# kouyt5/lightning-asr

Measured on AMD Instinct MI355X. Metric: audio-seconds/sec training (asr13x1, bs=32, 10 s clips), higher is better.
Workload: dtype bf16; 1 GPU; asr13x1 QuartzNet-CTC train step, bs=32/GPU, 10 s synthetic 16 kHz clips, labels.txt vocab (C=28), HIP mel+conv+CTC+NovoGrad, random-init weights; global_batch=32, n_class=28, parallelism=dp1, feature_prefetch=True, hip_graph=True, staged_backward=False

## Files before the change

include/lasr.h:

```cpp
#ifndef LASR_H
#define LASR_H

#include <stddef.h>
#include <stdint.h>

#ifdef __cplusplus
extern "C" {
#endif

#define LASR_VERSION 108

enum { LASR_F32 = 0, LASR_BF16 = 1 };
enum { LASR_ACT_NONE = 0, LASR_ACT_RELU = 1, LASR_ACT_SWISH = 2 };
enum { LASR_VARIANT_PLAIN = 0, LASR_VARIANT_CONTEXT = 1, LASR_VARIANT_CONTEXT_SE = 2 };
enum {
  LASR_E_ARG = -1,
  LASR_E_SHAPE = -2,
  LASR_E_WORKSPACE = -3,
  LASR_E_FORMAT = -4,
  LASR_E_UNSUPPORTED = -5,
  LASR_E_IO = -6
};

int lasr_version(void);
const char* lasr_last_error(void);

int64_t lasr_mel_num_frames(int64_t n_samples);
size_t lasr_mel_workspace_bytes(int64_t B, int64_t T);
int lasr_mel_fwd(const float* wave, const int32_t* sample_lens, const float* dither, const int32_t* aug,
                 int64_t B, int64_t L, int normalize, float* out_bft, void* out_btf, int dtype,
                 int32_t* frames_out, float* pct_out, void* workspace, size_t workspace_bytes, void* stream);

#define LASR_LEN_LEAD (1 << 30)
enum { LASR_WAVE_F32 = 0, LASR_WAVE_PCM16 = 1 };
typedef struct {
  const void* wave; int32_t wave_dtype; const float* dither; uint64_t dither_seed; uint64_t* dither_step; int64_t pitch;
} lasr_wave_src;
int lasr_mel_fwd_src(const lasr_wave_src* src, const int32_t* sample_lens, const int32_t* aug, int64_t B, int64_t L,
                     int normalize, float* out_bft, void* out_btf, int dtype, int32_t* frames_out, float* pct_out,
                     void* workspace, size_t workspace_bytes, void* stream);
int lasr_dither_noise(uint64_t seed, const uint64_t* step, int64_t B, int64_t L, float* out, void* stream);

int lasr_spec_augment(const float* in, float* out, const int32_t* aug, int64_t B, int64_t F, int64_t T, void* stream);

int lasr_bct_to_btc(const float* in, void* out, int dtype, int64_t B, int64_t C, int64_t T, void* stream);
int lasr_btc_to_bct(const void* in, int dtype, float* out, int64_t B, int64_t C, int64_t T, void* stream);

int lasr_mask_lengths(const float* pct, int64_t B, int64_t T, int32_t* lens, void* stream);


int lasr_dwconv_fwd(const void* x, const float* w, const void* addend, void* y, int dtype, int64_t B,
                    int64_t Tin, int64_t C, int k, int stride, int flip, void* stream);
size_t lasr_dwconv_wgrad_workspace_bytes(int64_t B, int64_t Tout, int64_t C, int k);
int lasr_dwconv_wgrad(const void* x, const void* dy, float* dw, int dtype, int64_t B, int64_t Tin,
                      int64_t C, int k, int stride, void* workspace, size_t workspace_bytes, void* stream);

size_t lasr_gemm_workspace_bytes(int64_t M, int64_t N, int split_k, int want_stats);
int lasr_gemm(const void* A, const void* B, void* C, int dtype_ab, int dtype_c, int64_t M, int64_t N,
              int64_t K, int transA, int transB, const float* bias, const void* addend,
              const int32_t* row_lens, int64_t rows_per_seq, float* stats, int split_k, void* workspace,
              size_t workspace_bytes, void* stream);

typedef struct {
  const void* A; const void* B; void* C;
  int64_t M, N, K;
  const float* bias; const int32_t* row_lens; int64_t rows_per_seq; float* stats;
} lasr_gemm_problem;
size_t lasr_gemm_batch_workspace_bytes(const lasr_gemm_problem* probs, int n_probs, int split_k);
int lasr_gemm_batch(const lasr_gemm_problem* probs, int n_probs, int dtype_ab, int dtype_c, int transA, int transB,
                    int split_k, void* workspace, size_t workspace_bytes, void* stream);

int lasr_gemm_ld(const void* A, int64_t lda, const void* B, int64_t ldb, void* C, int64_t ldc, int dtype_ab, int dtype_c,
                 int64_t M, int64_t N, int64_t K, int transA, int transB, const float* bias, int split_k, void* workspace,
                 size_t workspace_bytes, void* stream);

typedef struct {
  const float* w; const float* w_res; const float* coef; const float* coef2; void* w_out; float* bias_out; int64_t co, ci;
} lasr_fold_desc;
int lasr_fold_bn_weights_many(const lasr_fold_desc* descs, int n_descs, void* stream);
int lasr_gemm_dual(const void* A1, int64_t K1, const void* A2, int64_t K2, const void* W, const float* bias, void* C,
                   int64_t M, int64_t N, const int32_t* row_lens, int64_t rows_per_seq, int act, void* stream);

typedef struct { const float* partials; float* out; int64_t n; int32_t n_partials; } lasr_reduce_desc;
int lasr_reduce_many(const lasr_reduce_desc* descs, int n_descs, void* stream);
int lasr_gemm_batch_split_partials(const lasr_gemm_problem* probs, int n_probs, int dtype_ab, int transA, int transB,
                                   int split_k, void* workspace, size_t workspace_bytes, const float** partials,
                                   int* splits, void* stream);
int lasr_gemm_multi_split_partials(const lasr_gemm_problem* probs, int n_probs, int split_k, float* const* slabs,
                                   int* splits, void* stream);
int lasr_dwconv_wgrad_partials(const void* x, const void* dy, int dtype, int64_t B, int64_t Tin, int64_t C, int k,
                               int stride, void* workspace, size_t workspace_bytes, int* n_partials, void* stream);
int lasr_dwconv_bwd_fused(const void* x, const void* dy, const float* w, const void* addend, void* dx, int dtype,
                          int64_t B, int64_t T, int64_t C, int k, void* workspace, size_t workspace_bytes,
                          int* n_partials, void* stream);

int lasr_gemm_batch_partials(const lasr_gemm_problem* probs, int n_probs, int dtype_ab, int dtype_c, int transA,
                             int transB, void* workspace, size_t workspace_bytes, const float** stat_partials,
                             int* stat_tiles, void* stream);

int lasr_bn_finalize(const float* stats, const float* gamma, const float* beta, float* running_mean,
                     float* running_var, float* coef, float* saved, int64_t C, int64_t n_rows, float eps,
                     float momentum, int training, void* stream);
typedef struct {
  const float* gamma; const float* beta; const float* running_mean; const float* running_var; float* coef; int64_t C;
} lasr_bn_eval_desc;
int lasr_bn_eval_coef_many(const lasr_bn_eval_desc* descs, int n_descs, float eps, void* stream);

typedef struct {
  const float* partials; int n_partials;
  const float* gamma; const float* beta; float* running_mean; float* running_var;
  float* coef; float* saved; float* stats;
} lasr_bn_branch;
int lasr_bn_finalize_partials(const lasr_bn_branch* branches, int n_branches, int64_t C, int64_t n_rows, float eps,
                              float momentum, void* stream);
// ... 265 lines not shown
```

lightning_asr_amd/_lib.py:

```python
from __future__ import annotations

import ctypes as C
import os

_HERE = os.path.dirname(os.path.abspath(__file__))
LIB_PATH = os.environ.get("LASR_LIB_PATH", os.path.join(_HERE, "liblasr.so"))

F32, BF16 = 0, 1
ACT_NONE, ACT_RELU, ACT_SWISH = 0, 1, 2
LEN_LEAD = 1 << 30
VARIANT = {"plain": 0, "context": 1, "context_se": 2}

_p, _i64, _i32, _f32, _sz = C.c_void_p, C.c_int64, C.c_int, C.c_float, C.c_size_t


class Dropout(C.Structure):
    _fields_ = [("step", C.c_void_p), ("seed", C.c_uint64), ("unit", C.c_uint32), ("p", C.c_float)]


class WaveSrc(C.Structure):
    _fields_ = [("wave", C.c_void_p), ("wave_dtype", C.c_int32), ("dither", C.c_void_p), ("dither_seed", C.c_uint64),
                ("dither_step", C.c_void_p), ("pitch", C.c_int64)]


WAVE_F32, WAVE_PCM16 = 0, 1


class ModelConfig(C.Structure):
    _fields_ = [("variant", C.c_int32), ("n_class", C.c_int32), ("in_c", C.c_int32),
                ("mask", C.c_int32), ("act", C.c_int32), ("dtype", C.c_int32)]


SIGNATURES = {
    "lasr_version": (_i32, []),
    "lasr_roctx_range_push": (_i32, [C.c_char_p]),
    "lasr_roctx_range_pop": (_i32, []),
    "lasr_roctx_enabled": (_i32, []),
    "lasr_last_error": (C.c_char_p, []),
    "lasr_mel_num_frames": (_i64, [_i64]),
    "lasr_mel_workspace_bytes": (_sz, [_i64, _i64]),
    "lasr_mel_fwd": (_i32, [_p, _p, _p, _p, _i64, _i64, _i32, _p, _p, _i32, _p, _p, _p, _sz, _p]),
    "lasr_mel_fwd_src": (_i32, [_p, _p, _p, _i64, _i64, _i32, _p, _p, _i32, _p, _p, _p, _sz, _p]),
    "lasr_dither_noise": (_i32, [C.c_uint64, _p, _i64, _i64, _p, _p]),
    "lasr_spec_augment": (_i32, [_p, _p, _p, _i64, _i64, _i64, _p]),
    "lasr_bct_to_btc": (_i32, [_p, _p, _i32, _i64, _i64, _i64, _p]),
    "lasr_btc_to_bct": (_i32, [_p, _i32, _p, _i64, _i64, _i64, _p]),
    "lasr_mask_lengths": (_i32, [_p, _i64, _i64, _p, _p]),
    "lasr_dwconv_fwd": (_i32, [_p, _p, _p, _p, _i32, _i64, _i64, _i64, _i32, _i32, _i32, _p]),
    "lasr_dwconv_wgrad_workspace_bytes": (_sz, [_i64, _i64, _i64, _i32]),
    "lasr_dwconv_wgrad": (_i32, [_p, _p, _p, _i32, _i64, _i64, _i64, _i32, _i32, _p, _sz, _p]),
    "lasr_gemm_workspace_bytes": (_sz, [_i64, _i64, _i32, _i32]),
    "lasr_gemm": (_i32, [_p, _p, _p, _i32, _i32, _i64, _i64, _i64, _i32, _i32, _p, _p, _p, _i64, _p, _i32, _p, _sz, _p]),
    "lasr_gemm_batch_workspace_bytes": (_sz, [_p, _i32, _i32]),
    "lasr_gemm_batch": (_i32, [_p, _i32, _i32, _i32, _i32, _i32, _i32, _p, _sz, _p]),
    "lasr_bn_finalize": (_i32, [_p, _p, _p, _p, _p, _p, _p, _i64, _i64, _f32, _f32, _i32, _p]),
    "lasr_bn_eval_coef_many": (_i32, [_p, _i32, _f32, _p]),
    "lasr_bn_act_fwd": (_i32, [_p, _p, _p, _p, _p, _p, _i32, _i64, _i64, _i64, _i32, _p]),
    "lasr_bn_bwd_workspace_bytes": (_sz, [_i64, _i64, _i64]),
    "lasr_bn_act_bwd_stats": (_i32, [_p] * 11 + [_i32, _i64, _i64, _i64, _i32, _p, _sz, _p]),
    "lasr_bn_act_bwd_apply": (_i32, [_p] * 20 + [_i32, _i64, _i64, _i64, _i32, _p, _sz, _p]),
    "lasr_bn_bwd_apply_workspace_bytes": (_sz, [_i64]),
    "lasr_reduce_many": (_i32, [_p, _i32, _p]),
    "lasr_gemm_batch_split_partials": (_i32, [_p, _i32, _i32, _i32, _i32, _i32, _p, _sz, _p, _p, _p]),
    "lasr_gemm_multi_split_partials": (_i32, [_p, _i32, _i32, _p, _p, _p]),
    "lasr_dwconv_wgrad_partials": (_i32, [_p, _p, _i32, _i64, _i64, _i64, _i32, _i32, _p, _sz, _p, _p]),
    "lasr_dwconv_bwd_fused": (_i32, [_p, _p, _p, _p, _p, _i32, _i64, _i64, _i64, _i32, _p, _sz, _p, _p]),
    "lasr_gemm_batch_partials": (_i32, [_p, _i32, _i32, _i32, _i32, _i32, _p, _sz, _p, _p, _p]),
    "lasr_bn_finalize_partials": (_i32, [_p, _i32, _i64, _i64, C.c_float, C.c_float, _p]),
    "lasr_bn_act_fwd_partials": (_i32, [_p, _i32, C.c_float, C.c_float, _p, _p, _p, _i32, _i64, _i64, _i64, _i32, _p]),
    "lasr_seqsum": (_i32, [_p, _i32, _i64, _i64, _i64, _p, _p]),
    "lasr_se_fwd": (_i32, [_p, _p, _p, _p, _i64, _i64, _i64, _p, _p, _p, _p]),
    "lasr_se_bwd_workspace_bytes": (_sz, [_i64, _i64]),
    "lasr_se_bwd": (_i32, [_p] * 10 + [_i32, _i64, _i64, _i64, _i32, _p, _p, _p, _p, _sz, _p]),
    "lasr_bilstm_saved_bytes": (_sz, [_i64, _i64]),
    "lasr_bilstm_fwd": (_i32, [_p] * 9 + [_i64, _i64, _p, _i32, _i64, _i64, _p, _p]),
    "lasr_bilstm_bwd_workspace_bytes": (_sz, [_i64]),
    "lasr_bilstm_bwd": (_i32, [_p, _i32, _i64, _i64, _p, _p, _p, _i64, _i64, _p, _p, _p, _p, _p, _p, _sz, _p]),
    "lasr_copy_cols": (_i32, [_p, _i32, _i64, _i64, _p, _i32, _i64, _i64, _i64, _i64, _i32, _p]),
    "lasr_log_softmax": (_i32, [_p, _p, _p, _i64, _i64, _p]),
    "lasr_log_softmax_bwd": (_i32, [_p, _p, _p, _i64, _i64, _p]),
    "lasr_ctc_workspace_bytes": (_sz, [_i64, _i64, _i64]),
    "lasr_ctc_loss": (_i32, [_p, _p, _p, _p, _i64, _i64, _i64, _i64, _i32, _p, _p, _p, _p, _sz, _p]),
    "lasr_ctc_loss_mel": (_i32, [_p, _p, _p, _p, _i64, _i64, _i64, _i64, _i32, _p, _p, _p, _p, _sz,
                                 _p, _p, _p, _p, _i64, _i64, _i32, _p, _p, _i32, _p, _p, _p, _sz, _p]),
    "lasr_ctc_align_workspace_bytes": (_sz, [_i64, _i64, _i64]),
    "lasr_ctc_align": (_i32, [_p, _p, _p, _p, _i64, _i64, _i64, _i64, _i32, _p, _p, _p, _p, _p, _p, _sz, _p]),
    "lasr_greedy_decode": (_i32, [_p, _p, _i64, _i64, _i32, _p, _p, _p]),
    "lasr_ctc_beam_workspace_bytes": (_sz, [_i64, _i64, _i64, _i32, _i32]),
    "lasr_ctc_beam_decode": (_i32, [_p, _p, _i64, _i64, _i64, _i32, _i32, _i32, _f32, _i32, _p, _p, _p, _p, _sz, _p]),
    "lasr_arpa_load": (_i32, [C.c_char_p, _p, _i32, C.POINTER(_p)]),
    "lasr_arpa_info": (_i32, [_p, C.POINTER(C.c_int), C.POINTER(C.c_int), C.POINTER(_i64), C.POINTER(_sz)]),
    "lasr_arpa_write_image": (_i32, [_p, _p, _sz]),
    "lasr_arpa_free": (None, [_p]),
    "lasr_ctc_beam_lm_workspace_bytes": (_sz, [_i64, _i64, _i64, _i32, _i32]),
    "lasr_ctc_beam_decode_lm": (_i32, [_p, _p, _i64, _i64, _i64, _i32, _i32, _i32, _f32, _i32, _p, _f32, _f32, _p, _p, _p, _p, _p, _sz,
                                       _p]),
    "lasr_arpa_load_words": (_i32, [C.c_char_p, _p, _i32, _i32, C.POINTER(_p)]),
    "lasr_arpa_lexicon_info": (_i32, [_p, C.POINTER(_i64), C.POINTER(_i64), C.POINTER(_i64)]),
    "lasr_ctc_beam_decode_wlm": (_i32, [_p, _p, _i64, _i64, _i64, _i32, _i32, _i32, _f32, _i32, _p, _f32, _f32, _p, _p, _p, _p, _p, _sz,
                                        _p]),
    "lasr_novograd_workspace_bytes": (_sz, [_i64, _i64]),
    "lasr_novograd_step": (_i32, [_p, _p, _p, _p, _p, _i64, _i64, _p, _f32, _f32, _f32, _f32, _f32, _p, _sz, _p]),
    "lasr_novograd_step_keep": (_i32, [_p, _p, _p, _p, _p, _i64, _i64, _p, _f32, _f32, _f32, _f32, _f32, _p, _sz, _p]),
    "lasr_cast_f32_to_bf16": (_i32, [_p, _p, _i64, _p]),
    "lasr_cast_pad_f32_to_bf16": (_i32, [_p, _p, _i64, _i64, _i64, _p]),
# ... 105 lines not shown
```

lightning_asr_amd/csrc/gemm.h:

```cpp
#pragma once
#include "common.h"

namespace lasr {

struct GemmArgs {
  const void* A; const void* B; void* C;
  int64_t M, N, K, lda, ldb, ldc;
  const float* bias; const void* addend;
  const int32_t* row_lens; int64_t rows_per_seq;
  float* stat_partials;
  float* split_ws;
  int64_t k_per_split;
  int vecA, vecB;
};

int launch_gemm_bf16(const GemmArgs& g, int gz, int dtype_c, int transA, int transB, hipStream_t st, int* stat_tiles);
int launch_gemm_bf16_batch(const GemmArgs* g, const int* gz, int n, int dtype_c, int transA, int transB, hipStream_t st,
                           int* stat_tiles);

int launch_gemm_bf16_dual(const GemmArgs& g, const void* A2, int64_t lda2, int64_t K1, const float* bias, int act, hipStream_t st);
namespace lstm { struct BwdArgs; }
int launch_gemm_bf16_multi(const GemmArgs* g, const int* gz, int n, bool big_tile, hipStream_t st, const lstm::BwdArgs* lstm_job = nullptr,
                           int lstm_wgs = 0, const lasr_reduce_desc* riders = nullptr, int n_riders = 0, int* riders_taken = nullptr);
int gemm_multi_split_partials_riders(const lasr_gemm_problem* probs, int n_probs, int split_k, float* const* slabs, int* splits,
                                     const lasr_reduce_desc* riders, int n_riders, int* riders_taken, void* stream);
int gemm_split_partials_one(const void* A, const void* B, int dtype_ab, int64_t M, int64_t N, int64_t K, int transA, int transB, int split_k,
                            void* workspace, size_t workspace_bytes, int* splits, void* stream);
int gemm_multi_split_partials_with_bilstm_bwd(const lasr_gemm_problem* probs, int n_probs, int* n_taken, int split_k, float* const* slabs, int* splits,
                                              const lstm::BwdArgs& rec, int dtype, int64_t B, void* stream);
int launch_gemm_bf16_rowstat(const GemmArgs& g, float* row_stat, int32_t* row_arg, int* n_col_tiles, hipStream_t st);

}
```

lightning_asr_amd/csrc/gemm.hip:

```cpp
#include "common.h"
#include "gemm.h"
#include "lstm_body.h"
#include <cmath>
#include <climits>
#include <stdlib.h>

namespace lasr {

typedef float f32x16 __attribute__((ext_vector_type(16)));

static constexpr int BM = 128, BN = 128, BK = 16;
static constexpr int LDS_LD = BM + 4;

template <typename T, bool TRANS>
__device__ __forceinline__ void load_tile(const T* __restrict__ X, int64_t ld, int64_t R, int64_t K, int64_t r0, int64_t k0,
                                          int64_t kend, bool vec_ok, float (&reg)[2][4]) {
  const int tid = threadIdx.x;
#pragma unroll
  for (int p = 0; p < 2; ++p) {
    reg[p][0] = reg[p][1] = reg[p][2] = reg[p][3] = 0.f;
    if (!TRANS) {
      const int64_t r = r0 + (tid >> 2) + 64 * p;
      const int64_t k = k0 + ((tid & 3) << 2);
      if (r < R) {
// ... 169 lines not shown
                                                                int64_t ldc, const float* __restrict__ bias,
                                                                const TC* __restrict__ addend, TC* __restrict__ C) {
  const int64_t i = blockIdx.x * (int64_t)blockDim.x + threadIdx.x;
  if (i >= M * N) return;
  const int64_t m = i / N, n = i - m * N;
  float s = 0.f;
  for (int p = 0; p < split; ++p) s += ws[(int64_t)p * M * N + i];
  if (bias) s += bias[n];
  if (addend) s += Elem<TC>::ld(addend + m * ldc + n);
  Elem<TC>::st(C + m * ldc + n, s);
}

struct SplitReduce2 { const float* ws[2]; float* C[2]; const float* bias[2]; int split[2]; int64_t M[2], N[2]; };
__global__ __launch_bounds__(256) void gemm_split_reduce2_kernel(SplitReduce2 a) {
  const int q = blockIdx.y;
  const int64_t i = blockIdx.x * (int64_t)blockDim.x + threadIdx.x;
  const int64_t mn = a.M[q] * a.N[q];
  if (i >= mn) return;
  const float* ws = a.ws[q];
  float s = 0.f;
  for (int p = 0; p < a.split[q]; ++p) s += ws[(int64_t)p * mn + i];
  if (a.bias[q]) s += a.bias[q][i % a.N[q]];
  a.C[q][i] = s;
}

template <typename TAB, typename TC>
static int launch_f32(const GemmArgs& g, int transA, int transB, dim3 grid, hipStream_t st) {
#define LASR_GEMM_CASE(TA_, TB_)                                                                              \
  hipLaunchKernelGGL((gemm_f32_kernel<TAB, TC, TA_, TB_>), grid, dim3(256), 0, st, g)
  if (!transA && !transB) LASR_GEMM_CASE(false, false);
  else if (!transA && transB) LASR_GEMM_CASE(false, true);
  else if (transA && !transB) LASR_GEMM_CASE(true, false);
  else LASR_GEMM_CASE(true, true);
#undef LASR_GEMM_CASE
  LASR_LAUNCH_CHECK("gemm_f32_kernel");
  return 0;
}

}

using namespace lasr;

extern "C" size_t lasr_gemm_workspace_bytes(int64_t M, int64_t N, int split_k, int want_stats) {
  size_t b = 0;
  if (split_k > 1) b += align_up((size_t)split_k * M * N * sizeof(float), 256);
  if (want_stats) b += align_up((size_t)cdiv(M, BM) * 2 * N * sizeof(float), 256);
  return b;
}

struct StatOut { const float* partials; int tiles; };
static int gemm_impl(const void* A, const void* B, void* C, int dtype_ab, int dtype_c, int64_t M, int64_t N, int64_t K,
                     int transA, int transB, const float* bias, const void* addend, const int32_t* row_lens,
                     int64_t rows_per_seq, float* stats, int split_k, void* workspace, size_t workspace_bytes,
                     void* stream, StatOut* stat_out, int64_t lda = 0, int64_t ldb = 0, int64_t ldc = 0, int* split_left_out = nullptr) {
  LASR_CHECK_ARG(A && B && C, "lasr_gemm: null pointer");
  LASR_CHECK_ARG((dtype_ab == LASR_F32 || dtype_ab == LASR_BF16) && (dtype_c == LASR_F32 || dtype_c == LASR_BF16), "lasr_gemm: bad dtype");
  LASR_CHECK_SHAPE(M > 0 && N > 0 && K > 0 && split_k >= 1 && split_k <= 1024, "lasr_gemm: M=%lld N=%lld K=%lld split=%d",
                   (long long)M, (long long)N, (long long)K, split_k);
  LASR_CHECK_ARG(!(row_lens && rows_per_seq <= 0), "lasr_gemm: rows_per_seq");
  LASR_CHECK_ARG(!(split_k > 1 && (row_lens || stats)), "lasr_gemm: split_k excludes masking/statistics");
  const size_t need = lasr_gemm_workspace_bytes(M, N, split_k, stats != nullptr);
  if (need > 0 && (!workspace || workspace_bytes < need)) return fail(LASR_E_WORKSPACE, "lasr_gemm: workspace %zu < %zu", workspace_bytes, need);
  GemmArgs g;
  g.A = A; g.B = B; g.C = C; g.M = M; g.N = N; g.K = K;
  g.lda = lda > 0 ? lda : (transA ? M : K); g.ldb = ldb > 0 ? ldb : (transB ? N : K); g.ldc = ldc > 0 ? ldc : N;
  LASR_CHECK_SHAPE(g.lda >= (transA ? M : K) && g.ldb >= (transB ? N : K) && g.ldc >= N, "lasr_gemm: leading dimension smaller than the row");
  g.bias = bias; g.addend = addend; g.row_lens = row_lens; g.rows_per_seq = rows_per_seq;
  g.stat_partials = nullptr; g.split_ws = nullptr;
  const size_t esz = dtype_size(dtype_ab);
  const bool addend_ok = addend == nullptr || (dtype_c == LASR_BF16 && N % 4 == 0 && g.ldc % 4 == 0 && reinterpret_cast<uintptr_t>(addend) % 8 == 0);
  const bool use_bf16 = dtype_ab == LASR_BF16 && addend_ok && !getenv("LASR_FORCE_F32_MFMA");
  const int vw = use_bf16 ? 8 : 4;
  g.vecA = (g.lda % vw == 0) && (reinterpret_cast<uintptr_t>(A) % (vw * esz) == 0);
  g.vecB = (g.ldb % vw == 0) && (reinterpret_cast<uintptr_t>(B) % (vw * esz) == 0);
  char* wsp = reinterpret_cast<char*>(workspace);
  if (split_k > 1) {
    g.split_ws = reinterpret_cast<float*>(wsp);
    wsp += align_up((size_t)split_k * M * N * sizeof(float), 256);
    const int64_t per = cdiv(cdiv(K, split_k), 64) * 64;
    g.k_per_split = per;
    split_k = (int)cdiv(K, per);
  } else {
    g.k_per_split = K;
  }
  int grid_m = (int)cdiv(M, BM);
  if (stats) g.stat_partials = reinterpret_cast<float*>(wsp);
  dim3 grid((unsigned)cdiv(N, BN), (unsigned)grid_m, (unsigned)split_k);
  hipStream_t st = as_stream(stream);
  const double gbytes = (double)(M * K + N * K) * esz + (double)M * N * dtype_size(dtype_c);
  const int tok = prof_begin(LASR_PROF_GEMM, st, 2.0 * (double)M * (double)N * (double)K, gbytes);
  int rc;
  if (use_bf16) rc = launch_gemm_bf16(g, split_k, dtype_c, transA, transB, st, &grid_m);
  else if (dtype_ab == LASR_F32) rc = dtype_c == LASR_F32 ? launch_f32<float, float>(g, transA, transB, grid, st) : launch_f32<float, bf16_t>(g, transA, transB, grid, st);
  else rc = dtype_c == LASR_F32 ? launch_f32<bf16_t, float>(g, transA, transB, grid, st) : launch_f32<bf16_t, bf16_t>(g, transA, transB, grid, st);
  prof_end(tok, st);
  if (rc) return rc;
  if (g.split_ws && split_left_out) {
    *split_left_out = split_k;
  } else if (g.split_ws) {
    const int64_t mn = M * N;
    if (dtype_c == LASR_F32)
      hipLaunchKernelGGL(gemm_split_reduce_kernel<float>, dim3((unsigned)cdiv(mn, 256)), dim3(256), 0, st, g.split_ws, split_k, M, N, g.ldc, bias, (const float*)addend, (float*)C);
    else
      hipLaunchKernelGGL(gemm_split_reduce_kernel<bf16_t>, dim3((unsigned)cdiv(mn, 256)), dim3(256), 0, st, g.split_ws, split_k, M, N, g.ldc, bias, (const bf16_t*)addend, (bf16_t*)C);
    LASR_LAUNCH_CHECK("gemm_split_reduce_kernel");
  }
  if (stats && stat_out) {
    stat_out->partials = g.stat_partials; stat_out->tiles = grid_m;
  } else if (stats) {
    LASR_TRY(launch_reduce_partials(g.stat_partials, grid_m, 2 * N, stats, 2 * N, nullptr, st));
  }
  return 0;
}

int lasr::gemm_split_partials_one(const void* A, const void* B, int dtype_ab, int64_t M, int64_t N, int64_t K, int transA, int transB,
                                  int split_k, void* workspace, size_t workspace_bytes, int* splits, void* stream) {
  LASR_CHECK_ARG(splits && split_k > 1 && workspace, "gemm_split_partials_one: bad argument");
  return gemm_impl(A, B, workspace , dtype_ab, LASR_F32, M, N, K, transA, transB, nullptr, nullptr, nullptr,
                   0, nullptr, split_k, workspace, workspace_bytes, stream, nullptr, 0, 0, 0, splits);
}

extern "C" int lasr_gemm_ld(const void* A, int64_t lda, const void* B, int64_t ldb, void* C, int64_t ldc, int dtype_ab, int dtype_c,
                            int64_t M, int64_t N, int64_t K, int transA, int transB, const float* bias, int split_k, void* workspace,
                            size_t workspace_bytes, void* stream) {
  return gemm_impl(A, B, C, dtype_ab, dtype_c, M, N, K, transA, transB, bias, nullptr, nullptr, 0, nullptr, split_k, workspace,
                   workspace_bytes, stream, nullptr, lda, ldb, ldc);
}

extern "C" int lasr_gemm(const void* A, const void* B, void* C, int dtype_ab, int dtype_c, int64_t M, int64_t N, int64_t K,
                         int transA, int transB, const float* bias, const void* addend, const int32_t* row_lens,
                         int64_t rows_per_seq, float* stats, int split_k, void* workspace, size_t workspace_bytes,
                         void* stream) {
  return gemm_impl(A, B, C, dtype_ab, dtype_c, M, N, K, transA, transB, bias, addend, row_lens, rows_per_seq, stats, split_k,
                   workspace, workspace_bytes, stream, nullptr);
}

extern "C" int lasr_gemm_rowstat(const void* A, const void* B, const float* bias, void* C, int64_t ldc, int64_t M, int64_t N, int64_t K,
                                 float* row_stat, int32_t* row_arg, int* n_col_tiles, void* stream) {
  LASR_CHECK_ARG(A && B && C && row_stat && row_arg, "lasr_gemm_rowstat: null pointer");
  LASR_CHECK_SHAPE(M > 0 && N > 0 && K > 0 && K % 8 == 0 && ldc >= N && ldc % 8 == 0, "lasr_gemm_rowstat: M=%lld N=%lld K=%lld ldc=%lld",
                   (long long)M, (long long)N, (long long)K, (long long)ldc);
  GemmArgs g;
  g.A = A; g.B = B; g.C = C; g.M = M; g.N = N; g.K = K; g.lda = K; g.ldb = K; g.ldc = ldc;
  g.bias = bias; g.addend = nullptr; g.row_lens = nullptr; g.rows_per_seq = 0; g.stat_partials = nullptr; g.split_ws = nullptr;
  g.k_per_split = K;
  g.vecA = reinterpret_cast<uintptr_t>(A) % 16 == 0; g.vecB = reinterpret_cast<uintptr_t>(B) % 16 == 0;
  hipStream_t st = as_stream(stream);
  const int tok = prof_begin(LASR_PROF_GEMM, st, 2.0 * (double)M * N * K, (double)(M * K + N * K) * 2 + (double)M * N * 2);
  const int rc = launch_gemm_bf16_rowstat(g, row_stat, row_arg, n_col_tiles, st);
  prof_end(tok, st);
  return rc;
}
extern "C" size_t lasr_gemm_rowstat_bytes(int64_t M, int64_t N) { return (size_t)M * cdiv(N, 256) * (2 * sizeof(float) + sizeof(int32_t)); }

extern "C" size_t lasr_gemm_batch_workspace_bytes(const lasr_gemm_problem* probs, int n_probs, int split_k) {
  size_t b = 0;
  for (int i = 0; i < n_probs; ++i) b += lasr_gemm_workspace_bytes(probs[i].M, probs[i].N, split_k, probs[i].stats != nullptr);
  return b;
}

struct SplitOut { const float* partials; int splits; };
static int gemm_batch_impl(const lasr_gemm_problem* probs, int n_probs, int dtype_ab, int dtype_c, int transA, int transB,
                           int split_k, void* workspace, size_t workspace_bytes, void* stream, StatOut* stat_out,
                           SplitOut* split_out = nullptr) {
  LASR_CHECK_ARG(probs && n_probs >= 1 && n_probs <= 2, "lasr_gemm_batch: 1 or 2 problems");
  const size_t need = lasr_gemm_batch_workspace_bytes(probs, n_probs, split_k);
  if (need > 0 && (!workspace || workspace_bytes < need)) return fail(LASR_E_WORKSPACE, "lasr_gemm_batch: workspace %zu < %zu", workspace_bytes, need);
  char* wsp = reinterpret_cast<char*>(workspace);
  if (split_out && (dtype_ab != LASR_BF16 || n_probs == 1))
    return fail(LASR_E_ARG, "lasr_gemm_batch_split_partials: two bf16 problems per call");
  if (dtype_ab != LASR_BF16 || n_probs == 1 || getenv("LASR_NO_GEMM_BATCH")) {
    for (int i = 0; i < n_probs; ++i) {
      const lasr_gemm_problem& q = probs[i];
      const size_t nb = lasr_gemm_workspace_bytes(q.M, q.N, split_k, q.stats != nullptr);
      LASR_TRY(gemm_impl(q.A, q.B, q.C, dtype_ab, dtype_c, q.M, q.N, q.K, transA, transB, q.bias, nullptr, q.row_lens, q.rows_per_seq,
                         q.stats, split_k, wsp, nb, stream, stat_out ? stat_out + i : nullptr));
      wsp += nb;
    }
    return 0;
  }
  LASR_CHECK_ARG(dtype_c == LASR_F32 || dtype_c == LASR_BF16, "lasr_gemm_batch: bad dtype");
  GemmArgs g[2];
  int splits[2], stat_tiles[2];
  for (int i = 0; i < 2; ++i) {
    const lasr_gemm_problem& q = probs[i];
    LASR_CHECK_ARG(q.A && q.B && q.C, "lasr_gemm_batch: null pointer");
    LASR_CHECK_SHAPE(q.M > 0 && q.N > 0 && q.K > 0 && split_k >= 1 && split_k <= 1024, "lasr_gemm_batch: shape");
// ... 237 lines not shown
```

lightning_asr_amd/csrc/gemm_bf16.hip:

```cpp
#include "gemm.h"
#include "reduce_body.h"
#include "lstm_body.h"
#include <algorithm>
#include <stdlib.h>

namespace lasr {

__device__ __forceinline__ void load_bias_quads(const float* __restrict__ bias, int nbase, int N, float (&bv)[4][4]) {
#pragma unroll
  for (int ni = 0; ni < 4; ++ni)
#pragma unroll
    for (int e = 0; e < 4; ++e) {
      const int n = nbase + ni * 16 + e;
      bv[ni][e] = __uint_as_float(__float_as_uint(bias[min(n, N - 1)]) & (n < N ? 0xffffffffu : 0u));
    }
}


typedef float f32x4 __attribute__((ext_vector_type(4)));
typedef __bf16 bf16x8 __attribute__((ext_vector_type(8)));
typedef short s16x4 __attribute__((ext_vector_type(4)));
typedef short s16x8 __attribute__((ext_vector_type(8)));

static constexpr int TM = 128, TN = 128, TK = 64;
static constexpr int LD_KC = 144;
static constexpr int LD_RC = 320;
static constexpr int OPER_BYTES = 20480;
static constexpr int EPI_LD = 144;

union Frag { uint4 u; s16x8 s; bf16x8 b; };

struct Bf16Args {
  const bf16_t* A; const bf16_t* B; void* C;
  const float* bias; const int32_t* row_lens; float* stat_partials; float* split_ws;
  const bf16_t* addend;
  int M, N, K, lda, ldb, ldc, rows_per_seq, k_per_split;
  int gm, gn, gz;
  int vecA, vecB, vecC;
  const bf16_t* A2; int lda2, K1, act;
  float* row_stat; int32_t* row_arg;
};
struct Bf16Batch { Bf16Args p[2]; int tiles0, total; };

__device__ __forceinline__ int kc_slot(int row, int ch) { return ch ^ (((row >> 2) ^ (row >> 3)) & 1); }

__device__ __forceinline__ uint4 mask_chunk(const uint4& v, int nvalid) {
  const int n = max(0, min(nvalid, 8));
  if (n == 8) return v;
  auto dm = [n](int i) -> uint32_t { return n >= 2 * i + 2 ? 0xffffffffu : (n == 2 * i + 1 ? 0x0000ffffu : 0u); };
  return make_uint4(v.x & dm(0), v.y & dm(1), v.z & dm(2), v.w & dm(3));
}

template <bool TRANS, int ROWS, int NT, int NCH = 4, bool NTL = false>
// ... 733 lines not shown

template <bool NTL>
__global__ __launch_bounds__(512, 1) void gemm_bf16_big_multi_kernel(Bf16Multi gm) {
  if ((int)blockIdx.x >= gm.total) {
    const int r = blockIdx.x - gm.total;
    for (int s = 0; s < gm.n_rd; ++s) {
      const lasr_reduce_desc q = gm.rd[s];
      for (int64_t i = (int64_t)r * big::NT + threadIdx.x; i < q.n; i += (int64_t)gm.n_rwg * big::NT) reduce_many_elem(q, i);
    }
    return;
  }
  const int lid_all = xcd_remap(blockIdx.x, gm.total);
  int i = 0;
  while (i + 1 < gm.n && gm.start[i + 1] <= lid_all) ++i;
  gemm_bf16_big_tile<true, true, false, true, false, NTL>(gm.p[i], lid_all - gm.start[i]);
}

struct LstmJob { lstm::BwdArgs a; int n_wg; int n_utt; };
template <bool NTL, int KP, bool PAIR>
__global__ __launch_bounds__(512, 1) void gemm_bf16_big_multi_lstm_kernel(Bf16Multi gm, LstmJob job) {
  if ((int)blockIdx.x < job.n_wg) {
    __shared__ lstm::BwdSmem sm[2];
    const int slot = threadIdx.x / 192;
    if (slot >= (PAIR ? 2 : 1)) return;
    const int b = PAIR ? blockIdx.x : blockIdx.x >> 1, dir = PAIR ? slot : (blockIdx.x & 1);
    lstm::bilstm_bwd_body<bf16_t, true, KP>(job.a, b, dir, (int)threadIdx.x - slot * 192, 192, sm[slot], [] { lds_barrier(); });
    return;
  }
  const int lid_all = xcd_remap((int)blockIdx.x - job.n_wg, gm.total);
  int i = 0;
  while (i + 1 < gm.n && gm.start[i + 1] <= lid_all) ++i;
  gemm_bf16_big_tile<true, true, false, true, false, NTL>(gm.p[i], lid_all - gm.start[i]);
}

static int fill_args(Bf16Args& a, const GemmArgs& g, int tm, int tn, int gz) {
  const int64_t lim = (int64_t)1 << 31;
  const int64_t gn = cdiv(g.N, tn), gm = cdiv(g.M, tm);
  if (g.M * g.lda >= lim || g.K * g.lda >= lim || g.N * g.ldb >= lim || g.K * g.ldb >= lim || g.M * g.ldc >= lim ||
      gn * gm * gz >= lim / 2)
    return fail(LASR_E_SHAPE, "lasr_gemm(bf16): matrix exceeds the kernel's 32-bit element offsets");
  a.A = reinterpret_cast<const bf16_t*>(g.A); a.B = reinterpret_cast<const bf16_t*>(g.B); a.C = g.C;
  a.bias = g.bias; a.row_lens = g.row_lens; a.stat_partials = g.stat_partials; a.split_ws = g.split_ws;
  a.M = (int)g.M; a.N = (int)g.N; a.K = (int)g.K; a.lda = (int)g.lda; a.ldb = (int)g.ldb; a.ldc = (int)g.ldc;
  a.rows_per_seq = (int)(g.rows_per_seq > 0 ? g.rows_per_seq : 1); a.k_per_split = (int)g.k_per_split;
  a.gn = (int)gn; a.gm = (int)gm; a.gz = gz;
  a.vecA = g.vecA; a.vecB = g.vecB;
  a.vecC = (g.ldc % 8 == 0) && (reinterpret_cast<uintptr_t>(g.C) % 16 == 0);
  a.A2 = nullptr; a.lda2 = 0; a.K1 = 0; a.act = 0;
  a.row_stat = nullptr; a.row_arg = nullptr;
  a.addend = reinterpret_cast<const bf16_t*>(g.addend);
  return 0;
}

int launch_gemm_bf16_batch(const GemmArgs* g, const int* gz, int n, int dtype_c, int transA, int transB, hipStream_t st,
                           int* stat_tiles) {
  const bool f32_out = dtype_c == LASR_F32 || g[0].split_ws != nullptr;
  static const int big_min = getenv("LASR_GEMM_BIG_MIN_TILES") ? atoi(getenv("LASR_GEMM_BIG_MIN_TILES")) : 120;
  int64_t nmax = 0;
  for (int i = 0; i < n; ++i) nmax = std::max<int64_t>(nmax, g[i].N);
  static const bool force_narrow = getenv("LASR_GEMM_FORCE_NARROW") && atoi(getenv("LASR_GEMM_FORCE_NARROW")) != 0;
  const bool narrow = nmax <= 256 || force_narrow;
  const int btn = narrow ? 128 : 256;
  int64_t big_tiles = 0;
  for (int i = 0; i < n; ++i) big_tiles += cdiv(g[i].M, big::BTM) * cdiv(g[i].N, btn) * gz[i];
  bool vec = true;
  for (int i = 0; i < n; ++i) vec = vec && g[i].vecA && g[i].vecB;
  bool has_add = false;
  for (int i = 0; i < n; ++i) has_add = has_add || g[i].addend != nullptr;
  const bool use_big = !f32_out && vec && big_tiles >= big_min && !has_add;
  const int tm = use_big ? big::BTM : TM, tn = use_big ? btn : TN;
  Bf16Batch b;
  LASR_TRY(fill_args(b.p[0], g[0], tm, tn, gz[0]));
  b.p[1] = b.p[0];
  if (n > 1) LASR_TRY(fill_args(b.p[1], g[1], tm, tn, gz[1]));
  b.tiles0 = b.p[0].gn * b.p[0].gm * b.p[0].gz;
  b.total = b.tiles0 + (n > 1 ? b.p[1].gn * b.p[1].gm * b.p[1].gz : 0);
  if (stat_tiles)
    for (int i = 0; i < n; ++i) stat_tiles[i] = b.p[i].gm;
  const dim3 grid1((unsigned)b.total);
  if (use_big) {
#define LASR_BIG_CASE(TA_, TB_)                                                                              \
  do {                                                                                                     \
    if (narrow) hipLaunchKernelGGL((gemm_bf16_big_kernel<TA_, TB_, true>), grid1, dim3(big::NT), 0, st, b);  \
    else hipLaunchKernelGGL((gemm_bf16_big_kernel<TA_, TB_, false>), grid1, dim3(big::NT), 0, st, b);        \
  } while (0)
    if (!transA && !transB) LASR_BIG_CASE(false, false);
    else if (!transA && transB) LASR_BIG_CASE(false, true);
    else if (transA && !transB) LASR_BIG_CASE(true, false);
    else LASR_BIG_CASE(true, true);
#undef LASR_BIG_CASE
    LASR_LAUNCH_CHECK("gemm_bf16_big_kernel");
    return 0;
  }
#define LASR_BF16_CASE(TC_, TA_, TB_)                                                                    \
  do {                                                                                                  \
    if (vec) hipLaunchKernelGGL((gemm_bf16_kernel<TC_, TA_, TB_, true>), grid1, dim3(256), 0, st, b);    \
    else hipLaunchKernelGGL((gemm_bf16_kernel<TC_, TA_, TB_, false>), grid1, dim3(256), 0, st, b);       \
  } while (0)
#define LASR_BF16_TC(TC_)                                         \
  do {                                                            \
    if (!transA && !transB) LASR_BF16_CASE(TC_, false, false);    \
    else if (!transA && transB) LASR_BF16_CASE(TC_, false, true); \
    else if (transA && !transB) LASR_BF16_CASE(TC_, true, false); \
    else LASR_BF16_CASE(TC_, true, true);                         \
  } while (0)
  if (f32_out) LASR_BF16_TC(float); else LASR_BF16_TC(bf16_t);
#undef LASR_BF16_TC
#undef LASR_BF16_CASE
  LASR_LAUNCH_CHECK("gemm_bf16_kernel");
  return 0;
}

int launch_gemm_bf16_dual(const GemmArgs& g, const void* A2, int64_t lda2, int64_t K1, const float* bias, int act, hipStream_t st) {
  if (K1 <= 0 || K1 >= g.K || K1 % TK || (g.K - K1) % TK || lda2 % 8 || g.lda % 8 || g.ldb % 8 || g.ldc % 8 ||
      reinterpret_cast<uintptr_t>(g.A) % 16 || reinterpret_cast<uintptr_t>(A2) % 16 || reinterpret_cast<uintptr_t>(g.B) % 16 ||
      reinterpret_cast<uintptr_t>(g.C) % 16 || !bias)
    return fail(LASR_E_SHAPE, "lasr_gemm_dual: K parts must be multiples of %d, pitches of 8, pointers 16-byte aligned, bias given", TK);
  Bf16Batch b;
  LASR_TRY(fill_args(b.p[0], g, big::BTM, 128, 1));
  b.p[0].A2 = reinterpret_cast<const bf16_t*>(A2); b.p[0].lda2 = (int)lda2; b.p[0].K1 = (int)K1; b.p[0].act = act;
  b.p[0].bias = bias;
  b.p[1] = b.p[0];
  b.tiles0 = b.p[0].gn * b.p[0].gm;
  b.total = b.tiles0;
  hipLaunchKernelGGL(gemm_bf16_dual_kernel, dim3((unsigned)b.total), dim3(big::NT), 0, st, b);
  LASR_LAUNCH_CHECK("gemm_bf16_dual_kernel");
  return 0;
}

// ... 19 lines not shown
  Bf16Multi m;
  m.n_rd = 0; m.n_rwg = 0;
  bool vec = true;
  int total = 0;
  for (int i = 0; i < n; ++i) {
    if (!g[i].split_ws) return fail(LASR_E_ARG, "lasr_gemm_multi_split_partials: every problem needs a slab buffer");
    LASR_TRY(fill_args(m.p[i], g[i], big_tile ? big::BTM : TM, big_tile ? 256 : TN, gz[i]));
    vec = vec && g[i].vecA && g[i].vecB;
    m.start[i] = total;
    total += m.p[i].gn * m.p[i].gm * m.p[i].gz;
  }
  for (int i = n; i < kMaxMulti; ++i) m.p[i] = m.p[0];
  for (int i = n; i <= kMaxMulti; ++i) m.start[i] = total;
  m.n = n; m.total = total;
  if (big_tile) {
    if (!vec) return fail(LASR_E_ARG, "lasr_gemm_multi_split_partials: the 256-row tile needs 16-byte aligned operand rows");
    if (lstm_job) {
      static const bool pair = getenv("LASR_LSTM_PAIR") && atoi(getenv("LASR_LSTM_PAIR")) == 1;
      LstmJob job; job.a = *lstm_job; job.n_wg = lstm_wgs; job.n_utt = pair ? lstm_wgs : lstm_wgs / 2;
      if (job.n_wg % 8) return fail(LASR_E_SHAPE, "gemm + BiLSTM grid: the batch must be a multiple of 8 utterances");
      if (pair) hipLaunchKernelGGL((gemm_bf16_big_multi_lstm_kernel<false, 16, true>), dim3((unsigned)(total + job.n_wg)), dim3(big::NT), 0, st, m, job);
      else hipLaunchKernelGGL((gemm_bf16_big_multi_lstm_kernel<false, 16, false>), dim3((unsigned)(total + job.n_wg)), dim3(big::NT), 0, st, m, job);
      LASR_LAUNCH_CHECK("gemm_bf16_big_multi_lstm_kernel");
      return 0;
    }
    static const bool riders_off = getenv("LASR_WGRAD_RIDERS") && atoi(getenv("LASR_WGRAD_RIDERS")) == 0;
    const int idle = 256 - total;
    if (!riders_off && riders && riders_taken && n_riders > 0 && idle >= 8) {
      int ksteps = 0;
      for (int i = 0; i < n; ++i) ksteps = std::max(ksteps, (int)cdiv(m.p[i].k_per_split, 64));
      double budget = (double)idle * 20e9 * ((double)ksteps * 1.7e-6 + 20e-6) * 0.8;
      while (m.n_rd < n_riders && m.n_rd < kMaxRiders) {
        const lasr_reduce_desc& q = riders[m.n_rd];
        const double bytes = (double)q.n * (q.n_partials + 1) * sizeof(float);
        if (bytes > budget) break;
        budget -= bytes;
        m.rd[m.n_rd++] = q;
      }
      if (m.n_rd > 0) { m.n_rwg = idle; *riders_taken = m.n_rd; }
    }
    for (int i = m.n_rd; i < kMaxRiders; ++i) m.rd[i] = lasr_reduce_desc{nullptr, nullptr, 0, 0};
    if (nt_loads_mask() & 8) hipLaunchKernelGGL(gemm_bf16_big_multi_kernel<true>, dim3((unsigned)(total + m.n_rwg)), dim3(big::NT), 0, st, m);
    else hipLaunchKernelGGL(gemm_bf16_big_multi_kernel<false>, dim3((unsigned)(total + m.n_rwg)), dim3(big::NT), 0, st, m);
    LASR_LAUNCH_CHECK("gemm_bf16_big_multi_kernel");
    return 0;
  }
  if (lstm_job) return fail(LASR_E_SHAPE, "gemm + BiLSTM grid needs the 256-row tile form");
  if (vec) hipLaunchKernelGGL(gemm_bf16_multi_kernel<true>, dim3((unsigned)total), dim3(256), 0, st, m);
  else hipLaunchKernelGGL(gemm_bf16_multi_kernel<false>, dim3((unsigned)total), dim3(256), 0, st, m);
  LASR_LAUNCH_CHECK("gemm_bf16_multi_kernel");
  return 0;
}

int launch_gemm_bf16(const GemmArgs& g, int gz, int dtype_c, int transA, int transB, hipStream_t st, int* stat_tiles) {
  return launch_gemm_bf16_batch(&g, &gz, 1, dtype_c, transA, transB, st, stat_tiles);
}

}

#ifdef LASR_GEMM_STAMPS
extern "C" int lasr_debug_set_gemm_stamps(void* buf) {
  unsigned long long* p = reinterpret_cast<unsigned long long*>(buf);
  return (int)hipMemcpyToSymbol(HIP_SYMBOL(lasr::g_stamps), &p, sizeof(p));
}
#endif
```

Before: 160,300 audio-seconds/sec.

## Choose bf16 GEMM tile family with a wave-count cost model

Replaces the fixed heuristic for picking the GEMM tile shape (128x128, 256x128, 256x256), which used a tile-count threshold and an N cutoff, with a cost model. The model estimates waves over the device's CU count times per-tile fixed and per-K-step costs. It switches away from the old choice only when the predicted saving clears a margin, and it keeps the old choice for GEMMs that emit BN statistics. A new lasr_gemm_tile entry point allows forcing a tile family. The risk is that hand-fit cost constants may misjudge some shapes and pick a slower tile.

```diff
diff --git a/include/lasr.h b/include/lasr.h
--- a/include/lasr.h
+++ b/include/lasr.h
@@ -60,6 +60,9 @@
               int64_t K, int transA, int transB, const float* bias, const void* addend,
               const int32_t* row_lens, int64_t rows_per_seq, float* stats, int split_k, void* workspace,
               size_t workspace_bytes, void* stream);
+int lasr_gemm_tile(const void* A, const void* B, void* C, int dtype_ab, int dtype_c, int64_t M, int64_t N,
+                   int64_t K, int transA, int transB, const float* bias, const int32_t* row_lens,
+                   int64_t rows_per_seq, float* stats, int tile, void* workspace, size_t workspace_bytes, void* stream);
 
 typedef struct {
   const void* A; const void* B; void* C;
diff --git a/lightning_asr_amd/_lib.py b/lightning_asr_amd/_lib.py
--- a/lightning_asr_amd/_lib.py
+++ b/lightning_asr_amd/_lib.py
@@ -51,6 +51,7 @@
     "lasr_dwconv_wgrad": (_i32, [_p, _p, _p, _i32, _i64, _i64, _i64, _i32, _i32, _p, _sz, _p]),
     "lasr_gemm_workspace_bytes": (_sz, [_i64, _i64, _i32, _i32]),
     "lasr_gemm": (_i32, [_p, _p, _p, _i32, _i32, _i64, _i64, _i64, _i32, _i32, _p, _p, _p, _i64, _p, _i32, _p, _sz, _p]),
+    "lasr_gemm_tile": (_i32, [_p, _p, _p, _i32, _i32, _i64, _i64, _i64, _i32, _i32, _p, _p, _i64, _p, _i32, _p, _sz, _p]),
     "lasr_gemm_batch_workspace_bytes": (_sz, [_p, _i32, _i32]),
     "lasr_gemm_batch": (_i32, [_p, _i32, _i32, _i32, _i32, _i32, _i32, _p, _sz, _p]),
     "lasr_bn_finalize": (_i32, [_p, _p, _p, _p, _p, _p, _p, _i64, _i64, _f32, _f32, _i32, _p]),
diff --git a/lightning_asr_amd/csrc/gemm.h b/lightning_asr_amd/csrc/gemm.h
--- a/lightning_asr_amd/csrc/gemm.h
+++ b/lightning_asr_amd/csrc/gemm.h
@@ -14,9 +14,9 @@
   int vecA, vecB;
 };
 
-int launch_gemm_bf16(const GemmArgs& g, int gz, int dtype_c, int transA, int transB, hipStream_t st, int* stat_tiles);
+int launch_gemm_bf16(const GemmArgs& g, int gz, int dtype_c, int transA, int transB, hipStream_t st, int* stat_tiles, int force_tile = 0);
 int launch_gemm_bf16_batch(const GemmArgs* g, const int* gz, int n, int dtype_c, int transA, int transB, hipStream_t st,
-                           int* stat_tiles);
+                           int* stat_tiles, int force_tile = 0);
 
 int launch_gemm_bf16_dual(const GemmArgs& g, const void* A2, int64_t lda2, int64_t K1, const float* bias, int act, hipStream_t st);
 namespace lstm { struct BwdArgs; }
diff --git a/lightning_asr_amd/csrc/gemm.hip b/lightning_asr_amd/csrc/gemm.hip
--- a/lightning_asr_amd/csrc/gemm.hip
+++ b/lightning_asr_amd/csrc/gemm.hip
@@ -245,7 +245,8 @@
 static int gemm_impl(const void* A, const void* B, void* C, int dtype_ab, int dtype_c, int64_t M, int64_t N, int64_t K,
                      int transA, int transB, const float* bias, const void* addend, const int32_t* row_lens,
                      int64_t rows_per_seq, float* stats, int split_k, void* workspace, size_t workspace_bytes,
-                     void* stream, StatOut* stat_out, int64_t lda = 0, int64_t ldb = 0, int64_t ldc = 0, int* split_left_out = nullptr) {
+                     void* stream, StatOut* stat_out, int64_t lda = 0, int64_t ldb = 0, int64_t ldc = 0, int* split_left_out = nullptr,
+                     int force_tile = 0) {
   LASR_CHECK_ARG(A && B && C, "lasr_gemm: null pointer");
   LASR_CHECK_ARG((dtype_ab == LASR_F32 || dtype_ab == LASR_BF16) && (dtype_c == LASR_F32 || dtype_c == LASR_BF16), "lasr_gemm: bad dtype");
   LASR_CHECK_SHAPE(M > 0 && N > 0 && K > 0 && split_k >= 1 && split_k <= 1024, "lasr_gemm: M=%lld N=%lld K=%lld split=%d",
@@ -263,6 +264,7 @@
   const size_t esz = dtype_size(dtype_ab);
   const bool addend_ok = addend == nullptr || (dtype_c == LASR_BF16 && N % 4 == 0 && g.ldc % 4 == 0 && reinterpret_cast<uintptr_t>(addend) % 8 == 0);
   const bool use_bf16 = dtype_ab == LASR_BF16 && addend_ok && !getenv("LASR_FORCE_F32_MFMA");
+  LASR_CHECK_ARG(!force_tile || use_bf16, "lasr_gemm_tile: bf16 operands only");
   const int vw = use_bf16 ? 8 : 4;
   g.vecA = (g.lda % vw == 0) && (reinterpret_cast<uintptr_t>(A) % (vw * esz) == 0);
   g.vecB = (g.ldb % vw == 0) && (reinterpret_cast<uintptr_t>(B) % (vw * esz) == 0);
@@ -283,7 +285,7 @@
   const double gbytes = (double)(M * K + N * K) * esz + (double)M * N * dtype_size(dtype_c);
   const int tok = prof_begin(LASR_PROF_GEMM, st, 2.0 * (double)M * (double)N * (double)K, gbytes);
   int rc;
-  if (use_bf16) rc = launch_gemm_bf16(g, split_k, dtype_c, transA, transB, st, &grid_m);
+  if (use_bf16) rc = launch_gemm_bf16(g, split_k, dtype_c, transA, transB, st, &grid_m, force_tile);
   else if (dtype_ab == LASR_F32) rc = dtype_c == LASR_F32 ? launch_f32<float, float>(g, transA, transB, grid, st) : launch_f32<float, bf16_t>(g, transA, transB, grid, st);
   else rc = dtype_c == LASR_F32 ? launch_f32<bf16_t, float>(g, transA, transB, grid, st) : launch_f32<bf16_t, bf16_t>(g, transA, transB, grid, st);
   prof_end(tok, st);
@@ -326,6 +328,14 @@
                          void* stream) {
   return gemm_impl(A, B, C, dtype_ab, dtype_c, M, N, K, transA, transB, bias, addend, row_lens, rows_per_seq, stats, split_k,
                    workspace, workspace_bytes, stream, nullptr);
+}
+
+extern "C" int lasr_gemm_tile(const void* A, const void* B, void* C, int dtype_ab, int dtype_c, int64_t M, int64_t N, int64_t K,
+                              int transA, int transB, const float* bias, const int32_t* row_lens, int64_t rows_per_seq, float* stats,
+                              int tile, void* workspace, size_t workspace_bytes, void* stream) {
+  LASR_CHECK_ARG(tile >= 1 && tile <= 3, "lasr_gemm_tile: tile must be 1 (128 x 128), 2 (256 x 128) or 3 (256 x 256)");
+  return gemm_impl(A, B, C, dtype_ab, dtype_c, M, N, K, transA, transB, bias, nullptr, row_lens, rows_per_seq, stats, 1, workspace,
+                   workspace_bytes, stream, nullptr, 0, 0, 0, nullptr, tile);
 }
 
 extern "C" int lasr_gemm_rowstat(const void* A, const void* B, const float* bias, void* C, int64_t ldc, int64_t M, int64_t N, int64_t K,
diff --git a/lightning_asr_amd/csrc/gemm_bf16.hip b/lightning_asr_amd/csrc/gemm_bf16.hip
--- a/lightning_asr_amd/csrc/gemm_bf16.hip
+++ b/lightning_asr_amd/csrc/gemm_bf16.hip
@@ -1,4 +1,5 @@
 #include "gemm.h"
+#include "gemm_plan.h"
 #include "reduce_body.h"
 #include "lstm_body.h"
 #include <algorithm>
@@ -838,29 +839,55 @@
   return 0;
 }
 
+static const plan::Knobs& plan_knobs() {
+  static const plan::Knobs k = [] {
+    plan::Knobs q;
+    if (getenv("LASR_GEMM_BIG_MIN_TILES")) q.big_min = atoi(getenv("LASR_GEMM_BIG_MIN_TILES"));
+    q.force_narrow = getenv("LASR_GEMM_FORCE_NARROW") && atoi(getenv("LASR_GEMM_FORCE_NARROW")) != 0;
+    q.model = !(getenv("LASR_GEMM_PLAN") && atoi(getenv("LASR_GEMM_PLAN")) == 0);
+    return q;
+  }();
+  return k;
+}
+
+static int device_cus() {
+  static const int cus = [] {
+    int dev = 0, n = 0;
+    if (hipGetDevice(&dev) != hipSuccess || hipDeviceGetAttribute(&n, hipDeviceAttributeMultiprocessorCount, dev) != hipSuccess || n <= 0) n = 256;
+    return n;
+  }();
+  return cus;
+}
+
 int launch_gemm_bf16_batch(const GemmArgs* g, const int* gz, int n, int dtype_c, int transA, int transB, hipStream_t st,
-                           int* stat_tiles) {
+                           int* stat_tiles, int force_tile) {
   const bool f32_out = dtype_c == LASR_F32 || g[0].split_ws != nullptr;
-  static const int big_min = getenv("LASR_GEMM_BIG_MIN_TILES") ? atoi(getenv("LASR_GEMM_BIG_MIN_TILES")) : 120;
-  int64_t nmax = 0;
-  for (int i = 0; i < n; ++i) nmax = std::max<int64_t>(nmax, g[i].N);
-  static const bool force_narrow = getenv("LASR_GEMM_FORCE_NARROW") && atoi(getenv("LASR_GEMM_FORCE_NARROW")) != 0;
-  const bool narrow = nmax <= 256 || force_narrow;
-  const int btn = narrow ? 128 : 256;
-  int64_t big_tiles = 0;
-  for (int i = 0; i < n; ++i) big_tiles += cdiv(g[i].M, big::BTM) * cdiv(g[i].N, btn) * gz[i];
   bool vec = true;
   for (int i = 0; i < n; ++i) vec = vec && g[i].vecA && g[i].vecB;
   bool has_add = false;
   for (int i = 0; i < n; ++i) has_add = has_add || g[i].addend != nullptr;
-  const bool use_big = !f32_out && vec && big_tiles >= big_min && !has_add;
-  const int tm = use_big ? big::BTM : TM, tn = use_big ? btn : TN;
+  const bool big_ok = !f32_out && vec && !has_add;
+  plan::Problem pp[2];
+  for (int i = 0; i < n; ++i) pp[i] = {g[i].M, g[i].N, g[i].K, gz[i], g[i].stat_partials != nullptr};
+  plan::Plan pl = plan::make_plan(pp, n, big_ok, device_cus(), plan_knobs());
+  if (force_tile) {
+    if (force_tile < 1 || force_tile > 3 || (force_tile > 1 && !big_ok))
+      return fail(LASR_E_ARG, "lasr_gemm_tile: tile %d cannot run this problem (the 256-row tile needs a bf16 result and 16-byte aligned operands)", force_tile);
+    const plan::Family f = (plan::Family)(force_tile - 1);
+    pl.family = f; pl.tm = plan::tile_rows(f); pl.tn = plan::tile_cols(f); pl.workgroups = plan::workgroups(pp, n, f);
+    pl.fits = pl.workgroups < plan::kMaxGrid;
+  }
+  if (!pl.fits) return fail(LASR_E_SHAPE, "lasr_gemm(bf16): the launch exceeds the kernel's 32-bit tile indices");
+  const bool use_big = pl.family != plan::kTile128, narrow = pl.family == plan::kTile256x128;
+  const int tm = pl.tm, tn = pl.tn;
   Bf16Batch b;
   LASR_TRY(fill_args(b.p[0], g[0], tm, tn, gz[0]));
   b.p[1] = b.p[0];
   if (n > 1) LASR_TRY(fill_args(b.p[1], g[1], tm, tn, gz[1]));
   b.tiles0 = b.p[0].gn * b.p[0].gm * b.p[0].gz;
   b.total = b.tiles0 + (n > 1 ? b.p[1].gn * b.p[1].gm * b.p[1].gz : 0);
+  static_assert(TM == 128 && TN == 128 && big::BTM == 256 && big::NT == 512 && TK == plan::kStepK, "gemm_plan.h describes these tiles");
+  if (b.total != pl.workgroups) return fail(LASR_E_SHAPE, "lasr_gemm(bf16): the plan's grid (%lld) is not the launch's (%d)", (long long)pl.workgroups, b.total);
   if (stat_tiles)
     for (int i = 0; i < n; ++i) stat_tiles[i] = b.p[i].gm;
   const dim3 grid1((unsigned)b.total);
@@ -986,8 +1013,8 @@
   return 0;
 }
 
-int launch_gemm_bf16(const GemmArgs& g, int gz, int dtype_c, int transA, int transB, hipStream_t st, int* stat_tiles) {
-  return launch_gemm_bf16_batch(&g, &gz, 1, dtype_c, transA, transB, st, stat_tiles);
+int launch_gemm_bf16(const GemmArgs& g, int gz, int dtype_c, int transA, int transB, hipStream_t st, int* stat_tiles, int force_tile) {
+  return launch_gemm_bf16_batch(&g, &gz, 1, dtype_c, transA, transB, st, stat_tiles, force_tile);
 }
 
 }
diff --git a/lightning_asr_amd/csrc/gemm_plan.h b/lightning_asr_amd/csrc/gemm_plan.h
--- /dev/null
+++ b/lightning_asr_amd/csrc/gemm_plan.h
@@ -0,0 +1,110 @@
+#pragma once
+#include <algorithm>
+#include <cstdint>
+
+namespace lasr {
+namespace plan {
+
+enum Family { kTile128 = 0, kTile256x128 = 1, kTile256x256 = 2 };
+
+struct Problem {
+  int64_t M, N, K;
+  int slices;
+  bool stats;
+};
+
+struct Knobs {
+  int big_min = 120;
+  bool force_narrow = false;
+  bool model = true;
+};
+
+struct Plan {
+  Family family;
+  int tm, tn;
+  int threads;
+  int64_t workgroups;
+  double cost_us;
+  bool fits;
+};
+
+static constexpr double kStepWide = 1.7, kStepNarrow = 1.04, kStep128 = 1.7 * (1.3 / 0.7) / 2.0;
+static constexpr double kFixedWide = 1.8 + 5.2, kFixedNarrow = 5.4, kFixed128 = 3.7;
+static constexpr double kMargin = 0.15;
+static constexpr int kStepK = 64;
+static constexpr int64_t kMaxGrid = (int64_t)1 << 30;
+
+inline int64_t cdiv64(int64_t a, int64_t b) { return (a + b - 1) / b; }
+
+inline int tile_rows(Family f) { return f == kTile128 ? 128 : 256; }
+inline int tile_cols(Family f) { return f == kTile256x256 ? 256 : 128; }
+inline int tile_threads(Family f) { return f == kTile128 ? 256 : 512; }
+inline int slots_per_cu(Family f) { return f == kTile128 ? 2 : 1; }
+inline double step_us(Family f) { return f == kTile128 ? kStep128 : f == kTile256x128 ? kStepNarrow : kStepWide; }
+inline double fixed_us(Family f) { return f == kTile128 ? kFixed128 : f == kTile256x128 ? kFixedNarrow : kFixedWide; }
+
+inline int64_t workgroups(const Problem* p, int n, Family f) {
+  int64_t wg = 0;
+  for (int i = 0; i < n; ++i) wg += cdiv64(p[i].M, tile_rows(f)) * cdiv64(p[i].N, tile_cols(f)) * std::max(p[i].slices, 1);
+  return wg;
+}
+
+inline int64_t k_steps(const Problem* p, int n) {
+  int64_t ks = 1;
+  for (int i = 0; i < n; ++i) ks = std::max(ks, cdiv64(cdiv64(p[i].K, std::max(p[i].slices, 1)), kStepK));
+  return ks;
+}
+
+inline double cost_us(const Problem* p, int n, Family f, int cus) {
+  const int64_t slots = (int64_t)std::max(cus, 1) * slots_per_cu(f);
+  return (double)cdiv64(workgroups(p, n, f), slots) * (fixed_us(f) + (double)k_steps(p, n) * step_us(f));
+}
+
+inline bool admissible(const Problem* p, int n, Family f, bool big_ok, const Knobs& k) {
+  if (f == kTile128) return true;
+  if (!big_ok || (f == kTile256x256 && k.force_narrow)) return false;
+  return workgroups(p, n, f) >= k.big_min;
+}
+
+inline Family parent_family(const Problem* p, int n, bool big_ok, const Knobs& k) {
+  int64_t nmax = 0;
+  for (int i = 0; i < n; ++i) nmax = std::max(nmax, p[i].N);
+  const Family f = (nmax <= 256 || k.force_narrow) ? kTile256x128 : kTile256x256;
+  return admissible(p, n, f, big_ok, k) ? f : kTile128;
+}
+
+inline Family model_family(const Problem* p, int n, bool big_ok, int cus, const Knobs& k) {
+  const Family was = parent_family(p, n, big_ok, k);
+  for (int i = 0; i < n; ++i)
+    if (p[i].stats) return was;
+  Family best = was;
+  double best_cost = cost_us(p, n, was, cus) * (1.0 - kMargin);
+  for (int fi = kTile128; fi <= kTile256x256; ++fi) {
+    const Family f = (Family)fi;
+    if (f == was || !admissible(p, n, f, big_ok, k)) continue;
+    const double c = cost_us(p, n, f, cus);
+    if (c < best_cost) { best = f; best_cost = c; }
+  }
+  return best;
+}
+
+inline Plan make_plan(const Problem* p, int n, bool big_ok, int cus, const Knobs& k) {
+  Family f = k.model ? model_family(p, n, big_ok, cus, k) : parent_family(p, n, big_ok, k);
+  if (k.model && n > 1) {
+    bool any_stats = false;
+    for (int i = 0; i < n; ++i) any_stats = any_stats || p[i].stats;
+    for (int i = 0; i < n && !any_stats; ++i) {
+      const Family lone = model_family(p + i, 1, big_ok, cus, k);
+      if (lone > f && admissible(p, n, lone, big_ok, k)) f = lone;
+    }
+  }
+  Plan r;
+  r.family = f; r.tm = tile_rows(f); r.tn = tile_cols(f); r.threads = tile_threads(f);
+  r.workgroups = workgroups(p, n, f);
+  r.cost_us = k.model ? cost_us(p, n, f, cus) : 0.0;
+  r.fits = r.workgroups < kMaxGrid;
+  return r;
+}
+
+}
+}
```

After: 161,000 audio-seconds/sec, median of 6. About the same (+0.4%).
